# ramkp990/Truth_Recommendation_GNN

Measured on NVIDIA B200. Metric: message-passing edges/s (train step), higher is better.
Workload: dtype f32

## Files before the change

include/trg_b200.h:

```cpp
#ifndef TRG_B200_H
#define TRG_B200_H

#include <stddef.h>
#include <stdint.h>

#ifdef __cplusplus
extern "C" {
#endif

#define TRG_ABI_VERSION 4

enum { TRG_F32 = 0, TRG_BF16 = 1 };
enum {
  TRG_OK = 0,
  TRG_E_ARG = 1,
  TRG_E_WORKSPACE = 2,
  TRG_E_CUDA = 3,
  TRG_E_UNSUPPORTED = 4
};

int trg_abi_version(void);
const char* trg_last_error(void);
int64_t trg_launch_count(void);

// ... 44 lines not shown
size_t trg_edge_bce_workspace_bytes(int64_t n_users);
int trg_edge_bce_fwd(const int32_t* rowptr_u, const int32_t* col_p, const int32_t* eid,
                     const int64_t* neg_p, const void* u, const void* p,
                     int64_t n_users, int64_t n_edges, int32_t hidden, int dtype,
                     const float* wbar , float* loss_out,
                     float* c_pos, float* c_neg, void* g_u,
                     void* workspace, size_t workspace_bytes, void* stream);

int trg_edge_anchor_loss(const int32_t* rowptr, const int32_t* col, const int32_t* eid,
                         const void* anchor, const void* gathered, int64_t n_rows,
                         int64_t n_edges_scale, int32_t hidden, int dtype, int label,
                         const float* wbar, float* loss_out, float* coef_out, void* g_anchor,
                         int accumulate, int relu_gate, void* workspace, size_t workspace_bytes,
                         void* stream);

typedef struct {
  const void* a;
  const void* w;
  int32_t k;
  float alpha;
} trg_proj_term;
size_t trg_sage_proj_workspace_bytes(int32_t k_total, int32_t hidden, int dtype);
int trg_sage_proj_fwd(const trg_proj_term* terms , int32_t n_terms,
                      const float* bias ,
                      int64_t n_rows, int32_t hidden, int dtype, int relu,
                      void* out ,
                      void* workspace, size_t workspace_bytes, void* stream);

typedef struct {
  const void* w;
// ... 41 lines not shown
```

truth_recommendation_gnn_b200/_lib.py:

```python
from __future__ import annotations

import ctypes
import os

import torch

_HERE = os.path.dirname(os.path.abspath(__file__))
LIB_PATH = os.path.join(_HERE, "lib", "libtrg_b200.so")

TRG_F32, TRG_BF16 = 0, 1
ABI_VERSION = 4

_vp, _i64, _i32, _sz, _int = ctypes.c_void_p, ctypes.c_int64, ctypes.c_int32, ctypes.c_size_t, ctypes.c_int


class TrgProjTerm(ctypes.Structure):
    _fields_ = [("a", _vp), ("w", _vp), ("k", _i32), ("alpha", ctypes.c_float)]


class TrgLongRows(ctypes.Structure):
    _fields_ = [("vrowptr", _vp), ("vinfo", _vp), ("n_vrows", _i64), ("long_rows", _vp), ("long_ptr", _vp),
                ("n_long", _i64), ("partial", _vp)]


# ... 13 lines not shown
    "trg_csr_build": (_int, [_vp, _vp, _i64, _i64, _vp, _vp, _vp, _vp, _sz, _vp]),
    "trg_select_range_workspace_bytes": (_sz, [_i64]),
    "trg_select_range": (_int, [_vp, _vp, _i64, _i64, _i64, _i64, _i64, _i64, _vp, _vp, _vp, _vp, _sz, _vp]),
    "trg_sage_agg_fwd": (_int, [_vp, _vp, _vp, _i64, _i32, _int, _vp, _vp, ctypes.POINTER(TrgLongRows), _vp]),
    "trg_sage_agg_bwd": (_int, [_vp, _vp, _vp, _vp, _i64, _i32, _int, _vp, _int, _int, _vp,
                                ctypes.POINTER(TrgLongRows), _vp]),
    "trg_gather_wsum": (_int, [_vp, _vp, _vp, _vp, _vp, _vp, _i64, _i32, _int, _vp, _int, _int, _vp,
                               ctypes.POINTER(TrgLongRows), _vp]),
    "trg_rows_finish": (_int, [_vp, _int, _vp, _vp, _vp, _i64, _i32, _int, _vp, _vp]),
    "trg_peer_reduce_rows": (_int, [_vp, _i32, _i64, _int, _vp, _vp, _vp, _i64, _i32, _int, _vp, _i32, _vp]),
    "trg_edge_bce_workspace_bytes": (_sz, [_i64]),
    "trg_edge_bce_fwd": (_int, [_vp, _vp, _vp, _vp, _vp, _vp, _i64, _i64, _i32, _int, _vp, _vp,
                                _vp, _vp, _vp, _vp, _sz, _vp]),
    "trg_edge_anchor_loss": (_int, [_vp, _vp, _vp, _vp, _vp, _i64, _i64, _i32, _int, _int, _vp, _vp, _vp,
                                    _vp, _int, _int, _vp, _sz, _vp]),
    "trg_sage_proj_workspace_bytes": (_sz, [_i32, _i32, _int]),
    "trg_sage_proj_fwd": (_int, [ctypes.POINTER(TrgProjTerm), _i32, _vp, _i64, _i32, _int, _int, _vp,
                                 _vp, _sz, _vp]),
    "trg_sage_proj_bwd_input": (_int, [_vp, ctypes.POINTER(TrgProjBwdTerm), _i32, _i64, _i32, _int,
                                       _vp, _sz, _vp]),
    "trg_sage_proj_dw_workspace_bytes": (_sz, []),
    "trg_sage_proj_bwd_weight": (_int, [_vp, ctypes.POINTER(TrgProjDwTerm), _i32, _vp, _i64, _i32, _int,
                                        _vp, _sz, _vp]),
    "trg_score_topk_workspace_bytes": (_sz, [_i64, _i64, _i32, _i32]),
    "trg_score_topk": (_int, [_vp, _vp, _i64, _i64, _i32, _int, _i32, _i64, _vp, _vp, _vp, _sz, _vp]),
    "trg_score_topk_excluding": (_int, [_vp, _vp, _i64, _i64, _i32, _int, _i32, _i64, _vp, _vp, _vp, _vp, _vp,
                                        _vp, _sz, _vp]),
    "trg_topk_merge": (_int, [_vp, _vp, _i64, _i32, _i32, _i32, _vp, _vp, _vp]),
}

# ... 89 lines not shown
```

truth_recommendation_gnn_b200/csrc/csr_build.cu:

```cuda
#include <algorithm>
#include <cstdio>

#include "common.cuh"

namespace trg {
namespace {

constexpr int kThreads = 256;
constexpr int kItems = 16;
constexpr int kTile = kThreads * kItems;
constexpr int kWarps = kThreads / 32;
constexpr int kRadix = 256;

template <int NWARPS>
__device__ __forceinline__ int block_exclusive_scan(int v, int* warp_sums, int& total) {
  const int lane = threadIdx.x & 31, w = threadIdx.x >> 5;
  int inc = v;
#pragma unroll
  for (int o = 1; o < 32; o <<= 1) {
    int t = __shfl_up_sync(0xffffffffu, inc, o);
    if (lane >= o) inc += t;
  }
  if (lane == 31) warp_sums[w] = inc;
  __syncthreads();
// ... 184 lines not shown
  __shared__ int h[kRadix];
  h[threadIdx.x] = 0;
  __syncthreads();
  const int64_t base = (int64_t)blockIdx.x * kTile;
#pragma unroll
  for (int i = 0; i < kItems; ++i) {
    int64_t idx = base + (int64_t)i * kThreads + threadIdx.x;
    if (idx < n) atomicAdd(&h[(load_key<FIRST>(keys, idx) >> shift) & (kRadix - 1)], 1);
  }
  __syncthreads();
  hist[(int64_t)threadIdx.x * n_ctas + blockIdx.x] = h[threadIdx.x];
}

template <bool FIRST, bool LAST>
__global__ void __launch_bounds__(kThreads)
    radix_scatter(const void* __restrict__ keys_in, int64_t n, int shift, const int* __restrict__ gbase,
                  int n_ctas, uint2* __restrict__ pairs_out, uint32_t* __restrict__ vals_out) {
  __shared__ int wcnt[kWarps][kRadix];
  __shared__ int sbase[kRadix];
  const int lane = threadIdx.x & 31, w = threadIdx.x >> 5;
#pragma unroll
  for (int i = 0; i < kWarps; ++i) wcnt[i][threadIdx.x] = 0;
  const int64_t wbase = (int64_t)blockIdx.x * kTile + (int64_t)w * (kItems * 32);

  uint32_t key[kItems], val[kItems];
#pragma unroll
  for (int r = 0; r < kItems; ++r) {
    int64_t idx = wbase + r * 32 + lane;
    bool valid = idx < n;
    if (FIRST) {
      key[r] = valid ? load_key<true>(keys_in, idx) : 0u;
      val[r] = (uint32_t)idx;
    } else {
      const uint2 kv = valid ? ldg_pair(reinterpret_cast<const uint2*>(keys_in) + idx) : make_uint2(0u, 0u);
      key[r] = kv.x;
      val[r] = kv.y;
    }
  }
  __syncthreads();

  int rank[kItems];
#pragma unroll
  for (int r = 0; r < kItems; ++r) {
    const bool valid = wbase + r * 32 + lane < n;
    const int d = valid ? (int)((key[r] >> shift) & (kRadix - 1)) : kRadix;
    const unsigned peers = __match_any_sync(0xffffffffu, d);
    const int prev = valid ? wcnt[w][d] : 0;
// ... 31 lines not shown
                                                       const int* __restrict__ eid, int64_t n,
                                                       int* __restrict__ col) {
  int64_t i = (int64_t)blockIdx.x * blockDim.x + threadIdx.x;
  const int64_t stride = (int64_t)gridDim.x * blockDim.x;
  for (; i < n; i += stride) col[i] = (int)other[ldg_stream(eid + i)];
}

int num_passes(int64_t n_key) {
  int bits = 1;
  while (bits < 32 && ((int64_t)1 << bits) < n_key) ++bits;
  return (bits + 7) / 8;
}

struct Workspace {
  uint2* pairs[2];
  uint32_t* vals;
  int *hist, *tile_sums;
  size_t bytes;
};

Workspace carve(void* ws, int64_t e, int64_t n_key) {
  Workspace w;
  const size_t ebytes = align_up((size_t)(e > 0 ? e : 1) * 4, 256);
  const int64_t n_ctas = ceil_div<int64_t>(e > 0 ? e : 1, kTile);
  const size_t hist_bytes = align_up((size_t)kRadix * n_ctas * 4, 256);
  const int64_t scan_len = (int64_t)kRadix * n_ctas > n_key + 1 ? (int64_t)kRadix * n_ctas : n_key + 1;
  const size_t sums_bytes = align_up((size_t)ceil_div<int64_t>(scan_len, kTile) * 4 + 4, 256);
  char* p = reinterpret_cast<char*>(ws);
  w.pairs[0] = (uint2*)p; p += 2 * ebytes;
  w.pairs[1] = (uint2*)p; p += 2 * ebytes;
  w.vals = (uint32_t*)p; p += ebytes;
  w.hist = (int*)p; p += hist_bytes;
  w.tile_sums = (int*)p; p += sums_bytes;
  w.bytes = (size_t)(p - reinterpret_cast<char*>(ws));
  return w;
}

}
}

using namespace trg;

extern "C" size_t trg_csr_workspace_bytes(int64_t n_edges, int64_t n_key) {
  if (n_edges < 0 || n_key < 0) return 0;
  return carve(nullptr, n_edges, n_key).bytes;
}
// ... 20 lines not shown

  {
    int grid = (int)std::min<int64_t>(ceil_div<int64_t>(e, kThreads), (int64_t)kNumSMs * 16);
    count_keys<<<grid, kThreads, 0, st>>>((const long long*)key, e, (long long)n_key, rowptr);
    count_launch();
    TRG_LAUNCH_OK();
    int rc = exclusive_scan(rowptr, rowptr, n_key + 1, w.tile_sums, st);
    if (rc) return rc;
  }
  if (col == nullptr && eid == nullptr) return TRG_OK;

  const int passes = num_passes(n_key);
  const int n_ctas = (int)ceil_div<int64_t>(e, kTile);
  const void* kin = key;
  const uint32_t* vin = nullptr;
  for (int p = 0; p < passes; ++p) {
    const bool first = p == 0, last = p == passes - 1;
    const int shift = 8 * p;
    uint2* kout = w.pairs[p & 1];
    uint32_t* vout = eid ? (uint32_t*)eid : w.vals;
    if (first)
      radix_hist<true><<<n_ctas, kThreads, 0, st>>>(kin, e, shift, w.hist, n_ctas);
    else
      radix_hist<false><<<n_ctas, kThreads, 0, st>>>(kin, e, shift, w.hist, n_ctas);
    count_launch();
    TRG_LAUNCH_OK();
    int rc = exclusive_scan(w.hist, w.hist, (int64_t)kRadix * n_ctas, w.tile_sums, st);
    if (rc) return rc;
    if (first && last)
      radix_scatter<true, true><<<n_ctas, kThreads, 0, st>>>(kin, e, shift, w.hist, n_ctas, kout, vout);
    else if (first)
      radix_scatter<true, false><<<n_ctas, kThreads, 0, st>>>(kin, e, shift, w.hist, n_ctas, kout, vout);
    else if (last)
      radix_scatter<false, true><<<n_ctas, kThreads, 0, st>>>(kin, e, shift, w.hist, n_ctas, kout, vout);
    else
      radix_scatter<false, false><<<n_ctas, kThreads, 0, st>>>(kin, e, shift, w.hist, n_ctas, kout, vout);
    count_launch();
    TRG_LAUNCH_OK();
    kin = kout;
    vin = vout;
  }
  if (col != nullptr) {
    int grid = (int)std::min<int64_t>(ceil_div<int64_t>(e, kThreads), (int64_t)kNumSMs * 16);
    gather_col<<<grid, kThreads, 0, st>>>((const long long*)other, (const int*)vin, e, col);
    count_launch();
    TRG_LAUNCH_OK();
  }
  return TRG_OK;
}

extern "C" size_t trg_select_range_workspace_bytes(int64_t n) {
  if (n < 0) return 0;
  return align_up((size_t)(ceil_div<int64_t>(n > 0 ? n : 1, kTile) + 1) * 4, 256);
}

extern "C" int trg_select_range(const int64_t* key, const int64_t* other, int64_t n, int64_t lo, int64_t hi,
                                int64_t capacity, int64_t pad_key, int64_t pad_other, int64_t* key_out,
// ... 23 lines not shown
```

truth_recommendation_gnn_b200/csrc/edge_bce.cu:

```cuda
#include <cstdlib>

#include "common.cuh"

namespace trg {
namespace {

constexpr int kThreads = 256;

struct BceArgs {
  const int* rowptr;
  const int* col_p;
  const int* eid;
  const long long* neg_p;
  const void* u;
  const void* p;
  const float* wbar;
  float* c_pos;
  float* c_neg;
  void* g_u;
  double* partials;
  int64_t n_users;
  float inv_e;
  int row_vecs;
  int label;
// ... 186 lines not shown
#pragma unroll
              for (int i = 0; i < VPL; ++i)
                if (act[i]) {
                  float fp[kVec], fn[kVec];
                  Elem<T>::unpack(vp[q][i], fp);
                  if (TWO) Elem<T>::unpack(vn[q][i], fn);
#pragma unroll
                  for (int k = 0; k < kVec; ++k)
                    ga[i][k] = TWO ? fmaf(cpos, fp[k], fmaf(cneg, fn[k], ga[i][k])) : fmaf(cpos, fp[k], ga[i][k]);
                }
            }
          }
        }
        t += bsz;
      }
      if (want_grad && e0 + gl < e_end) {
        a.c_pos[id_cur] = my_cpos;
        if (TWO) a.c_neg[id_cur] = my_cneg;
      }
      e0 += LPR;
      cp_cur = cp_nxt; id_cur = id_nxt; cn_cur = cn_nxt;
      cp_nxt = cp_nn; id_nxt = id_nn;
    }
    while (cur < nr) flush();
  }

  double dsp = sp_sum, dsn = sn_sum;
#pragma unroll
  for (int o = 16; o > 0; o >>= 1) {
    dsp += __shfl_xor_sync(0xffffffffu, dsp, o);
    dsn += __shfl_xor_sync(0xffffffffu, dsn, o);
// ... 100 lines not shown
          cp_async16(ring_a + (uint32_t)(((slot0 + q) & (S - 1)) * 512), pb + (size_t)rid * 512 + (size_t)lane * 16);
      }
      cp_async_commit();
    };

    {
      const int id0 = load_id(e_beg), id1 = load_id(e_beg + G);
      issue(e_beg, id0, 0);
      issue(e_beg + G, id1, G);
    }
    int nid = load_id(e_beg + 2 * G);
    int slot = 0;
    for (int e_base = e_beg; e_base < e_end; e_base += G) {
      const int cnt = min(G, e_end - e_base);
      int my_id = 0;
      if (want_grad && lane < cnt) my_id = a.eid ? ldg_stream(a.eid + e_base + lane) : e_base + lane;
      cp_async_wait<1>();
      __syncwarp();
      float my_c = 0.f;
      int t = 0;
      while (t < cnt) {
        while (e_base + t >= cur_end) flush();
        const int bsz = min(cnt - t, cur_end - (e_base + t));
        uint4 vp[G];
        float v[G];
#pragma unroll
        for (int q = 0; q < G; ++q) {
          float dp = 0.f;
          if (q < bsz) {
            vp[q] = lds128_bce(ring_a + (uint32_t)(((slot + t + q) & (S - 1)) * 512));
            float fp[kVec];
// ... 30 lines not shown
          const float coef = (is_neg ? 1.f : -wbar) * sigmoid(z) * a.inv_e;
#pragma unroll
          for (int q = 0; q < G; ++q) {
            const float cq = __shfl_sync(full, coef, q * kLanesPerVal);
            if (q < bsz) {
              if (lane == t + q) my_c = cq;
              float fp[kVec];
              Elem<T>::unpack(vp[q], fp);
#pragma unroll
              for (int k = 0; k < kVec; ++k) ga[k] = fmaf(cq, fp[k], ga[k]);
            }
          }
        }
        t += bsz;
      }
      if (want_grad && lane < cnt) a.c_pos[my_id] = my_c;
      __syncwarp();
      const int nid_next = load_id(e_base + 3 * G);
      issue(e_base + 2 * G, nid, slot);
      nid = nid_next;
      slot = (slot + G) & (S - 1);
    }
    while (cur < nr) flush();
    cp_async_wait<0>();
  }

  double dsum = s_sum;
#pragma unroll
  for (int o = 16; o > 0; o >>= 1) dsum += __shfl_xor_sync(0xffffffffu, dsum, o);
  if (lane == 0) red[0][warp] = dsum;
  __syncthreads();
  if (threadIdx.x == 0) {
    double s0 = 0;
#pragma unroll
    for (int w = 0; w < kThreads / 32; ++w) s0 += red[0][w];
    const bool neg = a.label == 0;
    a.partials[2 * (size_t)blockIdx.x] = neg ? 0.0 : s0;
    a.partials[2 * (size_t)blockIdx.x + 1] = neg ? s0 : 0.0;
  }
}

__global__ void __launch_bounds__(1024) edge_bce_finish(const double* __restrict__ partials,
                                                        int64_t n_parts, const float* wbar,
                                                        double n_edges, float* loss_out) {
  __shared__ double red[2][32];
  double s0 = 0, s1 = 0;
  for (int64_t i = threadIdx.x; i < n_parts; i += 1024) {
    s0 += partials[2 * i];
    s1 += partials[2 * i + 1];
  }
#pragma unroll
  for (int o = 16; o > 0; o >>= 1) {
    s0 += __shfl_xor_sync(0xffffffffu, s0, o);
    s1 += __shfl_xor_sync(0xffffffffu, s1, o);
// ... 90 lines not shown
  edge_bce_finish<<<1, 1024, 0, st>>>(a.partials, n_blocks, wbar, (double)n_edges, loss_out);
  count_launch();
  TRG_LAUNCH_OK();
  return TRG_OK;
}

extern "C" int trg_edge_anchor_loss(const int32_t* rowptr, const int32_t* col, const int32_t* eid,
                                    const void* anchor, const void* gathered, int64_t n_rows,
                                    int64_t n_edges_scale, int32_t hidden, int dtype, int label,
                                    const float* wbar, float* loss_out, float* coef_out, void* g_anchor,
                                    int accumulate, int relu_gate, void* workspace, size_t workspace_bytes,
                                    void* stream) {
  cudaStream_t st = reinterpret_cast<cudaStream_t>(stream);
  TRG_CHECK_ARG(n_rows >= 0 && n_edges_scale >= 0, "trg_edge_anchor_loss: negative size");
  TRG_CHECK_ARG(loss_out && wbar, "trg_edge_anchor_loss: NULL loss_out/wbar");
  TRG_CHECK_ARG((coef_out == nullptr) == (g_anchor == nullptr),
                "trg_edge_anchor_loss: coef_out and g_anchor must be both NULL or both non-NULL");
  TRG_CHECK_ARG(n_rows == 0 || (rowptr && anchor), "trg_edge_anchor_loss: NULL rowptr / anchor table");
  TRG_CHECK_ARG(((uintptr_t)anchor | (uintptr_t)gathered | (uintptr_t)g_anchor) % 16 == 0,
                "trg_edge_anchor_loss: tables must be 16-byte aligned");
  TRG_CHECK_ARG(dtype == TRG_F32 || dtype == TRG_BF16, "trg_edge_anchor_loss: unknown dtype %d", dtype);
  const int es = dtype == TRG_BF16 ? 2 : 4;
  TRG_CHECK_ARG(hidden > 0 && (hidden * es) % 16 == 0,
                "trg_edge_anchor_loss: row width %d x %d bytes is not a multiple of 16 bytes", hidden, es);
  if (workspace == nullptr || workspace_bytes < trg_edge_bce_workspace_bytes(n_rows)) {
    set_error("trg_edge_anchor_loss: workspace %zu < required %zu", workspace_bytes,
              trg_edge_bce_workspace_bytes(n_rows));
    return TRG_E_WORKSPACE;
  }
  BceArgs a{};
  a.rowptr = rowptr; a.col_p = col; a.eid = eid; a.neg_p = nullptr;
  a.u = anchor; a.p = gathered; a.wbar = wbar; a.c_pos = coef_out; a.c_neg = nullptr; a.g_u = g_anchor;
// ... 17 lines not shown
    }
    count_launch();
    TRG_LAUNCH_OK();
  } else if (n_rows > 0) {
    int rc = dtype == TRG_F32 ? launch_bce<float, false>(a, &n_blocks, st, false)
                              : launch_bce<__nv_bfloat16, false>(a, &n_blocks, st, false);
    if (rc) return rc;
    count_launch();
    TRG_LAUNCH_OK();
  }
  edge_bce_finish<<<1, 1024, 0, st>>>(a.partials, n_blocks, wbar, (double)n_edges_scale, loss_out);
  count_launch();
  TRG_LAUNCH_OK();
  return TRG_OK;
}
```

truth_recommendation_gnn_b200/functional.py:

```python
from __future__ import annotations

import ctypes

import torch

from . import _lib
from .graph import CSR, RelationGraph, build_csr


def _long_rows_arg(csr: CSR, feat: int, dev, elem_size: int = 4):
    lr = csr.long_rows() if feat * elem_size >= 80 else None
    if lr is None:
        return None, None
    partial = torch.empty(lr.n_slots, feat, dtype=torch.float32, device=dev)
    s = _lib.TrgLongRows(_lib.ptr(lr.vrowptr), _lib.ptr(lr.vinfo), int(lr.vinfo.numel()), _lib.ptr(lr.long_rows),
                         _lib.ptr(lr.long_ptr), int(lr.long_rows.numel()), _lib.ptr(partial))
    return ctypes.byref(s), (s, partial)


def _check_rows(x: torch.Tensor, what: str):
    es = x.element_size()
    if x.dim() != 2 or (x.size(1) * es) % 16 != 0:
        raise _lib.TrgError(f"{what}: rows must be a multiple of 16 bytes (got shape {tuple(x.shape)}, "
                            f"{x.dtype}); pad the feature width (the reference pads to 64, inference.py:401-404)")
# ... 219 lines not shown
    ws = torch.empty(ws_bytes, dtype=torch.uint8, device=dev)
    e = ls.n_edges
    e_scale = int(getattr(ls, "n_edges_scale", e))
    rb = user_emb.size(1) * user_emb.element_size()
    nbytes = e * (2 * rb + 16 + (8 if want_grad else 0)) + ls.num_users * (rb * (2 if want_grad else 1) + 4)
    _lib.call("trg_edge_bce_fwd", nbytes, lib.trg_edge_bce_fwd,
              _lib.ptr(ls.by_user.rowptr), _lib.ptr(ls.by_user.col) if e else None,
              _lib.ptr(ls.by_user.eid) if e else None, _lib.ptr(neg_p) if e else None,
              _lib.ptr(user_emb), _lib.ptr(post_emb), ls.num_users, e_scale, user_emb.size(1),
              _lib.dtype_code(user_emb.dtype), _lib.ptr(ls.wbar), _lib.ptr(loss), _lib.ptr(c_pos),
              _lib.ptr(c_neg), _lib.ptr(g_u), _lib.ptr(ws), ws_bytes, _lib.stream())
    return loss, c_pos, c_neg, g_u


def edge_anchor_loss(csr: CSR, anchor, gathered, n_edges_scale, label, wbar, want_grad, g_anchor=None,
                     relu_gate=False, coef_in_csr_order=False):
    lib = _lib.load()
    anchor, gathered = anchor.contiguous(), gathered.contiguous()
    _check_rows(anchor, "edge_anchor_loss")
    dev = anchor.device
    loss = torch.empty(1, dtype=torch.float32, device=dev)
    coef = None
    accumulate = g_anchor is not None
    if want_grad:
        coef = torch.empty(csr.n_edges, dtype=torch.float32, device=dev)
        if g_anchor is None:
            g_anchor = torch.empty_like(anchor)
    else:
        g_anchor = None
    ws_bytes = int(lib.trg_edge_bce_workspace_bytes(csr.n_rows))
    ws = torch.empty(ws_bytes, dtype=torch.uint8, device=dev)
    e = csr.n_edges
    rb = anchor.size(1) * anchor.element_size()
    nbytes = e * (rb + 12) + csr.n_rows * (rb * (2 if want_grad else 1) + 4)
    _lib.call("trg_edge_anchor_loss", nbytes, lib.trg_edge_anchor_loss,
              _lib.ptr(csr.rowptr), _lib.ptr(csr.col) if e else None,
              _lib.ptr(csr.eid) if (e and not coef_in_csr_order) else None,
              _lib.ptr(anchor), _lib.ptr(gathered), csr.n_rows, int(n_edges_scale), anchor.size(1),
              _lib.dtype_code(anchor.dtype), 1 if label else 0, _lib.ptr(wbar), _lib.ptr(loss), _lib.ptr(coef),
              _lib.ptr(g_anchor), 1 if (accumulate and want_grad) else 0,
              1 if (relu_gate and want_grad) else 0, _lib.ptr(ws), ws_bytes, _lib.stream())
    return loss, coef, g_anchor


class LinkBCEFn(torch.autograd.Function):

    @staticmethod
    def forward(ctx, user_emb, post_emb, neg_p, ls: LinkStructure):
        want = user_emb.requires_grad or post_emb.requires_grad
        if neg_p.dtype != torch.int64 or neg_p.numel() != ls.n_edges:
            raise _lib.TrgError("neg_p must be int64 with one entry per positive edge (train_gnn.py:272)")
        if getattr(ls, "eid_long", None) is None:
            ls.eid_long = ls.by_user.eid.long()
        e_scale = int(getattr(ls, "n_edges_scale", ls.n_edges))
        bu = ls.by_user
        ctx.neg_by_post = None
        if want and ls.n_edges:
# ... 205 lines not shown
```

truth_recommendation_gnn_b200/fused_step.py:

```python
from __future__ import annotations

import torch

from . import _lib
from .functional import (edge_anchor_loss, gather_wsum, link_structure, sage_agg_bwd, sage_agg_fwd,
                         sage_proj_bwd_input, sage_proj_bwd_weight, sage_proj_fwd)
from .graph import CSR, build_csr, relation_graph
from .nn import REL_DIRECT, REL_ENGAGE, REL_SOCIAL, StackedWeightedRGCN, WeightedRGCN


def _layers(model):
    if type(model) is StackedWeightedRGCN:
        return list(model.layers)
    if type(model) is WeightedRGCN:
        return [model]
    return None


def eligible(model, x_dict) -> bool:
    layers = _layers(model)
    if layers is None or not torch.is_grad_enabled():
        return False
    xu, xp = x_dict["user"], x_dict["post"]
    if not (xu.is_cuda and xp.is_cuda) or xu.requires_grad or xp.requires_grad or xu.dtype != xp.dtype:
# ... 46 lines not shown
        hu_n = sage_proj_fwd([(mean_d, d.lin_l.weight, wd), (mean_s, s.lin_l.weight, ws), (hu, w_root, 1.0)],
                             b_user, True)
        hp_n = sage_proj_fwd([(mean_e, p.lin_l.weight, 1.0), (hp, p.lin_r.weight, 1.0)], p.lin_l.bias, True)
        saved.append((hu, hp, mean_d, mean_s, mean_e, w_root))
        hu, hp = hu_n, hp_n

    ls = link_structure(train_edge_index, interaction_type_tensor, num_users, n_p)
    if neg_ready is not None:
        torch.cuda.current_stream().wait_event(neg_ready)
    if neg_p.dtype != torch.int64 or neg_p.numel() != ls.n_edges:
        raise _lib.TrgError("neg_p must be int64 with one entry per positive edge (train_gnn.py:272)")
    if getattr(ls, "eid_long", None) is None:
        ls.eid_long = ls.by_user.eid.long()
    bu = ls.by_user
    col_neg64 = neg_p.index_select(0, ls.eid_long)
    neg_by_post = build_csr(ls.user_of_u, col_neg64, n_p, n_u, validate=False, per_step=True)
    neg_by_user = CSR(bu.rowptr, col_neg64.int(), bu.eid, bu.n_rows, bu.n_cols)
    l_pos, c_pos, dz_u = edge_anchor_loss(bu, hu, hp, ls.n_edges, 1, ls.wbar, True, None, coef_in_csr_order=True)
    l_neg, c_neg, dz_u = edge_anchor_loss(neg_by_user, hu, hp, ls.n_edges, 0, ls.wbar, True, dz_u,
                                          relu_gate=True, coef_in_csr_order=True)
    dz_p = gather_wsum(ls.by_post_u, c_pos, hu)
    gather_wsum(neg_by_post, c_neg, hu, out=dz_p, accumulate=True, relu_of=hp)
    del col_neg64
    loss = (l_pos + l_neg).reshape(())
    del neg_by_user, neg_by_post, c_pos, c_neg, hu, hp

    for li in range(len(layers) - 1, -1, -1):
        layer = layers[li]
        d, s, p = layer.msg_direct, layer.msg_social, layer.post_update
        wd, ws = float(layer.w_direct), float(layer.w_social)
        hu_in, hp_in, mean_d, mean_s, mean_e, w_root = saved.pop()
        (dw_d, dw_s, dw_root), db_u = sage_proj_bwd_weight(dz_u, [(mean_d, wd), (mean_s, ws), (hu_in, 1.0)], True)
        (dw_p, dw_pr), db_p = sage_proj_bwd_weight(dz_p, [(mean_e, 1.0), (hp_in, 1.0)], True)
        del mean_d, mean_s, mean_e
        _accum(d.lin_l.weight, dw_d)
        _accum(s.lin_l.weight, dw_s)
        _accum(d.lin_r.weight, wd * dw_root)
        _accum(s.lin_r.weight, ws * dw_root)
# ... 17 lines not shown
```

truth_recommendation_gnn_b200/graph.py:

```python
from __future__ import annotations

from collections import OrderedDict
from dataclasses import dataclass

import torch

from . import _lib


LONG_ROW_THRESHOLD = 1024


@dataclass
class LongRows:
    vrowptr: torch.Tensor
    vinfo: torch.Tensor
    long_rows: torch.Tensor
    long_ptr: torch.Tensor
    n_slots: int


@dataclass
class CSR:
    rowptr: torch.Tensor
    col: torch.Tensor
    eid: torch.Tensor
    n_rows: int
    n_cols: int
    _long: object = None

    @property
    def n_edges(self) -> int:
        return int(self.col.numel())

    def long_rows(self, threshold: int = None):
        if self._long is None:
            self._long = _split_long_rows(self, LONG_ROW_THRESHOLD if threshold is None else threshold) or False
        return self._long or None


def _split_long_rows(csr: "CSR", t: int):
# ... 10 lines not shown
    vstart = torch.cumsum(counts, 0) - counts
    k = torch.arange(n_vrows, device=rp.device) - vstart[orig]
    vrowptr = torch.empty(n_vrows + 1, dtype=torch.int32, device=rp.device)
    vrowptr[:-1] = (rp[:-1][orig] + k * t).int()
    vrowptr[-1] = csr.n_edges
    part = is_long[orig]
    slot = torch.cumsum(part.long(), 0) - 1
    vinfo = torch.where(part, -(slot + 1), orig).int()
    long_ids = is_long.nonzero().flatten()
    lp = torch.zeros(long_ids.numel() + 1, dtype=torch.long, device=rp.device)
    lp[1:] = torch.cumsum(counts[long_ids], 0)
    return LongRows(vrowptr, vinfo, long_ids.int(), lp.int(), int(lp[-1]))


def build_csr(other: torch.Tensor, key: torch.Tensor, n_key: int, n_other: int,
              validate: bool = True, per_step: bool = False) -> CSR:
    lib = _lib.load()
    if key.dtype != torch.int64 or other.dtype != torch.int64:
        raise TypeError("edge_index must be int64 (torch.long), as in the reference")
    key = key.contiguous()
    other = other.contiguous()
    e = int(key.numel())
    dev = key.device
    if validate and e > 0:
        lo_k, hi_k = int(key.min()), int(key.max())
        lo_o, hi_o = int(other.min()), int(other.max())
        if lo_k < 0 or hi_k >= n_key or lo_o < 0 or hi_o >= n_other:
            raise IndexError(f"edge_index out of range: key in [{lo_k},{hi_k}] vs {n_key}, "
                             f"other in [{lo_o},{hi_o}] vs {n_other}")
    rowptr = torch.empty(n_key + 1, dtype=torch.int32, device=dev)
    col = torch.empty(e, dtype=torch.int32, device=dev)
    eid = torch.empty(e, dtype=torch.int32, device=dev)
    ws_bytes = int(lib.trg_csr_workspace_bytes(e, n_key))
    ws = torch.empty(ws_bytes, dtype=torch.uint8, device=dev)
    _lib.call("trg_csr_build", e * 80 + 8 * (n_key + 1), lib.trg_csr_build,
              _lib.ptr(other) if e else None, _lib.ptr(key) if e else None, e, n_key, _lib.ptr(rowptr),
              _lib.ptr(col) if e else None, _lib.ptr(eid) if e else None, _lib.ptr(ws), ws_bytes,
              _lib.stream())
    return CSR(rowptr, col, eid, n_key, n_other, False if per_step else None)


class RelationGraph:

    def __init__(self, edge_index: torch.Tensor, n_src: int, n_dst: int):
        if edge_index.dim() != 2 or edge_index.size(0) != 2:
            raise ValueError("edge_index must have shape [2, E]")
        self.edge_index = edge_index
        self.n_src, self.n_dst = int(n_src), int(n_dst)
        self._fwd = None
        self._bwd = None
        self.inv_deg = None

# ... 55 lines not shown
```

Before: 2.956 billion.

## Fuse post-side link BCE gradient into one pass recomputing scores

Adds a link_post_grad kernel that walks each post's positive and negative user edges, recomputes the dot-product scores, and accumulates the weighted user rows with the ReLU gate applied in a single pass. This replaces two gather_wsum calls and removes the need to write and read per-edge coefficient arrays. The per-step negative CSR build now carries the column as the radix payload and skips the eid output and the gather_col pass. The cost is recomputing scores on the post side and a path that only applies to 512-byte rows.

Measured after the change: 3.023 billion (median of 6 runs). 1.02x the previous value.

```diff
diff --git a/include/trg_b200.h b/include/trg_b200.h
--- a/include/trg_b200.h
+++ b/include/trg_b200.h
@@ -82,6 +82,12 @@
                          int accumulate, int relu_gate, void* workspace, size_t workspace_bytes,
                          void* stream);
 
+int trg_link_post_grad(const int32_t* pos_rowptr, const int32_t* pos_col, const int32_t* neg_rowptr,
+                       const int32_t* neg_col, const void* hp, const void* hu, int64_t n_posts,
+                       int64_t n_edges_scale, int32_t hidden, int dtype, const float* wbar ,
+                       void* dz_p ,
+                       const trg_long_rows* long_rows , void* stream);
+
 typedef struct {
   const void* a;
   const void* w;
diff --git a/truth_recommendation_gnn_b200/_lib.py b/truth_recommendation_gnn_b200/_lib.py
--- a/truth_recommendation_gnn_b200/_lib.py
+++ b/truth_recommendation_gnn_b200/_lib.py
@@ -51,6 +51,8 @@
                                 _vp, _vp, _vp, _vp, _sz, _vp]),
     "trg_edge_anchor_loss": (_int, [_vp, _vp, _vp, _vp, _vp, _i64, _i64, _i32, _int, _int, _vp, _vp, _vp,
                                     _vp, _int, _int, _vp, _sz, _vp]),
+    "trg_link_post_grad": (_int, [_vp, _vp, _vp, _vp, _vp, _vp, _i64, _i64, _i32, _int, _vp, _vp,
+                                  ctypes.POINTER(TrgLongRows), _vp]),
     "trg_sage_proj_workspace_bytes": (_sz, [_i32, _i32, _int]),
     "trg_sage_proj_fwd": (_int, [ctypes.POINTER(TrgProjTerm), _i32, _vp, _i64, _i32, _int, _int, _vp,
                                  _vp, _sz, _vp]),
diff --git a/truth_recommendation_gnn_b200/csrc/csr_build.cu b/truth_recommendation_gnn_b200/csrc/csr_build.cu
--- a/truth_recommendation_gnn_b200/csrc/csr_build.cu
+++ b/truth_recommendation_gnn_b200/csrc/csr_build.cu
@@ -222,8 +222,9 @@
 
 template <bool FIRST, bool LAST>
 __global__ void __launch_bounds__(kThreads)
-    radix_scatter(const void* __restrict__ keys_in, int64_t n, int shift, const int* __restrict__ gbase,
-                  int n_ctas, uint2* __restrict__ pairs_out, uint32_t* __restrict__ vals_out) {
+    radix_scatter(const void* __restrict__ keys_in, const long long* __restrict__ payload, int64_t n, int shift,
+                  const int* __restrict__ gbase, int n_ctas, uint2* __restrict__ pairs_out,
+                  uint32_t* __restrict__ vals_out) {
   __shared__ int wcnt[kWarps][kRadix];
   __shared__ int sbase[kRadix];
   const int lane = threadIdx.x & 31, w = threadIdx.x >> 5;
@@ -238,7 +239,7 @@
     bool valid = idx < n;
     if (FIRST) {
       key[r] = valid ? load_key<true>(keys_in, idx) : 0u;
-      val[r] = (uint32_t)idx;
+      val[r] = payload ? (valid ? (uint32_t)ldg_stream(payload + idx) : 0u) : (uint32_t)idx;
     } else {
       const uint2 kv = valid ? ldg_pair(reinterpret_cast<const uint2*>(keys_in) + idx) : make_uint2(0u, 0u);
       key[r] = kv.x;
@@ -300,7 +301,6 @@
 
 struct Workspace {
   uint2* pairs[2];
-  uint32_t* vals;
   int *hist, *tile_sums;
   size_t bytes;
 };
@@ -315,7 +315,6 @@
   char* p = reinterpret_cast<char*>(ws);
   w.pairs[0] = (uint2*)p; p += 2 * ebytes;
   w.pairs[1] = (uint2*)p; p += 2 * ebytes;
-  w.vals = (uint32_t*)p; p += ebytes;
   w.hist = (int*)p; p += hist_bytes;
   w.tile_sums = (int*)p; p += sums_bytes;
   w.bytes = (size_t)(p - reinterpret_cast<char*>(ws));
@@ -366,11 +365,12 @@
   const int n_ctas = (int)ceil_div<int64_t>(e, kTile);
   const void* kin = key;
   const uint32_t* vin = nullptr;
+  const long long* payload = eid ? nullptr : (const long long*)other;
   for (int p = 0; p < passes; ++p) {
     const bool first = p == 0, last = p == passes - 1;
     const int shift = 8 * p;
     uint2* kout = w.pairs[p & 1];
-    uint32_t* vout = eid ? (uint32_t*)eid : w.vals;
+    uint32_t* vout = eid ? (uint32_t*)eid : (uint32_t*)col;
     if (first)
       radix_hist<true><<<n_ctas, kThreads, 0, st>>>(kin, e, shift, w.hist, n_ctas);
     else
@@ -380,19 +380,19 @@
     int rc = exclusive_scan(w.hist, w.hist, (int64_t)kRadix * n_ctas, w.tile_sums, st);
     if (rc) return rc;
     if (first && last)
-      radix_scatter<true, true><<<n_ctas, kThreads, 0, st>>>(kin, e, shift, w.hist, n_ctas, kout, vout);
+      radix_scatter<true, true><<<n_ctas, kThreads, 0, st>>>(kin, payload, e, shift, w.hist, n_ctas, kout, vout);
     else if (first)
-      radix_scatter<true, false><<<n_ctas, kThreads, 0, st>>>(kin, e, shift, w.hist, n_ctas, kout, vout);
+      radix_scatter<true, false><<<n_ctas, kThreads, 0, st>>>(kin, payload, e, shift, w.hist, n_ctas, kout, vout);
     else if (last)
-      radix_scatter<false, true><<<n_ctas, kThreads, 0, st>>>(kin, e, shift, w.hist, n_ctas, kout, vout);
+      radix_scatter<false, true><<<n_ctas, kThreads, 0, st>>>(kin, payload, e, shift, w.hist, n_ctas, kout, vout);
     else
-      radix_scatter<false, false><<<n_ctas, kThreads, 0, st>>>(kin, e, shift, w.hist, n_ctas, kout, vout);
+      radix_scatter<false, false><<<n_ctas, kThreads, 0, st>>>(kin, payload, e, shift, w.hist, n_ctas, kout, vout);
     count_launch();
     TRG_LAUNCH_OK();
     kin = kout;
     vin = vout;
   }
-  if (col != nullptr) {
+  if (col != nullptr && eid != nullptr) {
     int grid = (int)std::min<int64_t>(ceil_div<int64_t>(e, kThreads), (int64_t)kNumSMs * 16);
     gather_col<<<grid, kThreads, 0, st>>>((const long long*)other, (const int*)vin, e, col);
     count_launch();
diff --git a/truth_recommendation_gnn_b200/csrc/edge_bce.cu b/truth_recommendation_gnn_b200/csrc/edge_bce.cu
--- a/truth_recommendation_gnn_b200/csrc/edge_bce.cu
+++ b/truth_recommendation_gnn_b200/csrc/edge_bce.cu
@@ -224,7 +224,7 @@
         }
         t += bsz;
       }
-      if (want_grad && e0 + gl < e_end) {
+      if (a.c_pos && e0 + gl < e_end) {
         a.c_pos[id_cur] = my_cpos;
         if (TWO) a.c_neg[id_cur] = my_cneg;
       }
@@ -355,7 +355,7 @@
     for (int e_base = e_beg; e_base < e_end; e_base += G) {
       const int cnt = min(G, e_end - e_base);
       int my_id = 0;
-      if (want_grad && lane < cnt) my_id = a.eid ? ldg_stream(a.eid + e_base + lane) : e_base + lane;
+      if (a.c_pos && lane < cnt) my_id = a.eid ? ldg_stream(a.eid + e_base + lane) : e_base + lane;
       cp_async_wait<1>();
       __syncwarp();
       float my_c = 0.f;
@@ -416,7 +416,7 @@
         }
         t += bsz;
       }
-      if (want_grad && lane < cnt) a.c_pos[my_id] = my_c;
+      if (a.c_pos && lane < cnt) a.c_pos[my_id] = my_c;
       __syncwarp();
       const int nid_next = load_id(e_base + 3 * G);
       issue(e_base + 2 * G, nid, slot);
@@ -440,6 +440,311 @@
     a.partials[2 * (size_t)blockIdx.x] = neg ? 0.0 : s0;
     a.partials[2 * (size_t)blockIdx.x + 1] = neg ? s0 : 0.0;
   }
+}
+
+struct PostGradArgs {
+  const int* pos_rowptr;
+  const int* vinfo;
+  const int* pos_col;
+  const int* neg_rowptr;
+  const int* neg_col;
+  const void* hp;
+  const void* hu;
+  const float* wbar;
+  void* dz_p;
+  float* partial;
+  const int* long_rows;
+  const int* long_ptr;
+  int n_long;
+  int64_t n_vrows;
+  float inv_e;
+};
+
+template <typename T>
+constexpr int kPgG = sizeof(T) == 4 ? 4 : 2;
+constexpr int kPgSlots = 12;
+constexpr int kPgR = 4;
+constexpr int kPgBytes = (kThreads / 32) * (kPgSlots + 1) * 512;
+
+template <typename T, int G>
+__device__ __forceinline__ float batch_scores(const uint4* vr, int bsz, const float* af) {
+  constexpr int kVec = Elem<T>::kVec;
+  const int lane = threadIdx.x & 31;
+  float v[G];
+#pragma unroll
+  for (int q = 0; q < G; ++q) {
+    float dp = 0.f;
+    if (q < bsz) {
+      float f[kVec];
+      Elem<T>::unpack(vr[q], f);
+#pragma unroll
+      for (int k = 0; k < kVec; ++k) dp = fmaf(f[k], af[k], dp);
+    }
+    v[q] = dp;
+  }
+  int nv = G;
+#pragma unroll
+  for (int o = 16; o > 0; o >>= 1) {
+    if (nv > 1) {
+      nv >>= 1;
+#pragma unroll
+      for (int i = 0; i < G / 2; ++i) {
+        if (i < nv) {
+          const bool hi = (lane & o) != 0;
+          const float send = hi ? v[i] : v[i + nv];
+          const float keep = hi ? v[i + nv] : v[i];
+          v[i] = keep + __shfl_xor_sync(0xffffffffu, send, o);
+        }
+      }
+    } else {
+      v[0] += __shfl_xor_sync(0xffffffffu, v[0], o);
+    }
+  }
+  return v[0];
+}
+
+__device__ __forceinline__ float link_coef(float s, bool neg, float wbar, float inv_e) {
+  const float z = neg ? s : -s;
+  return (neg ? 1.f : -wbar) * sigmoid(z) * inv_e;
+}
+
+template <typename T>
+__device__ __forceinline__ void post_grad_store(char* dst, const float* an, const float* pr, const float* af) {
+  constexpr int kVec = Elem<T>::kVec;
+  float o[kVec];
+#pragma unroll
+  for (int k = 0; k < kVec; ++k) {
+    o[k] = an[k] + pr[k];
+    o[k] = af[k] > 0.f ? o[k] : 0.f;
+  }
+  stg_stream(dst, Elem<T>::pack(o));
+}
+
+template <typename T, bool VIRT>
+__global__ void __launch_bounds__(kThreads, 4) link_post_grad(const PostGradArgs a) {
+  constexpr int kVec = Elem<T>::kVec;
+  constexpr int R = kPgR, G = kPgG<T>, S = kPgSlots, NG = S / G;
+  constexpr int kLanesPerVal = 32 / G;
+  constexpr unsigned full = 0xffffffffu;
+  extern __shared__ __align__(16) unsigned char ring_raw[];
+  const int lane = threadIdx.x & 31, warp = threadIdx.x >> 5;
+  const int64_t r0 = ((int64_t)blockIdx.x * (kThreads / 32) + warp) * R;
+  if (r0 >= a.n_vrows) return;
+  const uint32_t smem0 = static_cast<uint32_t>(__cvta_generic_to_shared(ring_raw));
+  const uint32_t ring_a = smem0 + (uint32_t)(warp * S * 512 + lane * 16);
+  const uint32_t pos_a = smem0 + (uint32_t)(((kThreads / 32) * S + warp) * 512 + lane * 16);
+  const int nr = (int)((a.n_vrows - r0) < (int64_t)R ? (a.n_vrows - r0) : (int64_t)R);
+  const char* hpb = reinterpret_cast<const char*>(a.hp);
+  const char* hub = reinterpret_cast<const char*>(a.hu);
+  const float wbar = __ldg(a.wbar);
+
+  int pb = 0, np = 0, nb = 0, nn = 0, info = 0, arow = 0;
+  if (lane < nr) {
+    pb = ldg_stream(a.pos_rowptr + r0 + lane);
+    np = ldg_stream(a.pos_rowptr + r0 + lane + 1) - pb;
+    info = VIRT ? ldg_stream(a.vinfo + r0 + lane) : (int)(r0 + lane);
+    if (info >= 0) {
+      nb = ldg_stream(a.neg_rowptr + info);
+      nn = ldg_stream(a.neg_rowptr + info + 1) - nb;
+      arow = info;
+    } else {
+      const int slot = -(info + 1);
+      int lo = 0, hi = a.n_long - 1;
+      while (lo < hi) {
+        const int mid = (lo + hi + 1) >> 1;
+        if (__ldg(a.long_ptr + mid) <= slot) lo = mid; else hi = mid - 1;
+      }
+      arow = __ldg(a.long_rows + lo);
+    }
+  }
+  int inc = np + nn;
+#pragma unroll
+  for (int o = 1; o < R; o <<= 1) {
+    const int t = __shfl_up_sync(full, inc, o);
+    if (lane >= o) inc += t;
+  }
+  const int e_end = __shfl_sync(full, inc, nr - 1);
+  const int cs = lane < nr ? inc - (np + nn) : e_end;
+
+  auto row_lane = [&](int m, int v) { return __shfl_sync(full, v, m); };
+  auto load_id = [&](int ebase) -> int {
+    const int e = ebase + lane;
+    int r = 0;
+#pragma unroll
+    for (int m = 1; m < R; ++m)
+      if (e >= row_lane(m, cs)) r = m;
+    const int off = e - row_lane(r, cs);
+    const int npr = row_lane(r, np), pbr = row_lane(r, pb), nbr = row_lane(r, nb);
+    if (lane >= G || e >= e_end) return 0;
+    return off < npr ? ldg_stream(a.pos_col + pbr + off) : ldg_stream(a.neg_col + nbr + (off - npr));
+  };
+  auto issue = [&](int ebase, int ids, int slot0) {
+#pragma unroll
+    for (int q = 0; q < G; ++q) {
+      const int rid = __shfl_sync(full, ids, q);
+      if (ebase + q < e_end)
+        cp_async16(ring_a + (uint32_t)((slot0 + q) * 512), hub + (size_t)rid * 512 + (size_t)lane * 16);
+    }
+    cp_async_commit();
+  };
+
+  float af[kVec], acc[kVec];
+#pragma unroll
+  for (int k = 0; k < kVec; ++k) acc[k] = 0.f;
+  Elem<T>::unpack(ldg_row(hpb + (size_t)row_lane(0, arow) * 512 + (size_t)lane * 16), af);
+  uint4 a_nxt = make_uint4(0, 0, 0, 0);
+  {
+    const int ar1 = row_lane(1, arow);
+    if (nr > 1) a_nxt = ldg_row(hpb + (size_t)ar1 * 512 + (size_t)lane * 16);
+  }
+  int cur = 0;
+  int cur_end = row_lane(1, cs);
+  int pos_end = row_lane(0, np);
+  bool in_neg = false;
+
+  auto flush = [&]() {
+    const int inf = row_lane(cur, info);
+    if (VIRT && inf < 0) {
+      float* pbp = a.partial + (size_t)(-(inf + 1)) * (32 * kVec) + (size_t)lane * kVec;
+#pragma unroll
+      for (int k = 0; k < kVec; ++k) pbp[k] = acc[k];
+    } else {
+      float pr[kVec], an[kVec];
+      if (in_neg) {
+        Elem<T>::unpack(lds128_bce(pos_a), pr);
+#pragma unroll
+        for (int k = 0; k < kVec; ++k) an[k] = acc[k];
+      } else {
+        Elem<T>::unpack(Elem<T>::pack(acc), pr);
+#pragma unroll
+        for (int k = 0; k < kVec; ++k) an[k] = 0.f;
+      }
+      post_grad_store<T>(reinterpret_cast<char*>(a.dz_p) + (size_t)inf * 512 + (size_t)lane * 16, an, pr, af);
+    }
+#pragma unroll
+    for (int k = 0; k < kVec; ++k) acc[k] = 0.f;
+    in_neg = false;
+    ++cur;
+    pos_end = cur_end + row_lane(cur, np);
+    cur_end = row_lane(cur + 1, cs);
+    Elem<T>::unpack(a_nxt, af);
+    const int arn = row_lane(cur + 1, arow);
+    if (cur + 1 < nr) a_nxt = ldg_row(hpb + (size_t)arn * 512 + (size_t)lane * 16);
+  };
+
+#pragma unroll
+  for (int g = 0; g < NG; ++g) issue(g * G, load_id(g * G), g * G);
+  int nid = load_id(NG * G);
+  int slot = 0;
+  for (int e_base = 0; e_base < e_end; e_base += G) {
+    const int cnt = min(G, e_end - e_base);
+    cp_async_wait<NG - 1>();
+    __syncwarp();
+    int t = 0;
+    while (t < cnt) {
+      const int e = e_base + t;
+      while (e >= cur_end) flush();
+      if (!in_neg && e >= pos_end) {
+        const uint4 pk = Elem<T>::pack(acc);
+        asm volatile("st.shared.v4.u32 [%0], {%1,%2,%3,%4};" ::"r"(pos_a), "r"(pk.x), "r"(pk.y), "r"(pk.z),
+                     "r"(pk.w) : "memory");
+#pragma unroll
+        for (int k = 0; k < kVec; ++k) acc[k] = 0.f;
+        in_neg = true;
+      }
+      const int bsz = min(cnt - t, (in_neg ? cur_end : pos_end) - e);
+      uint4 vr[G];
+#pragma unroll
+      for (int q = 0; q < G; ++q)
+        if (q < bsz) vr[q] = lds128_bce(ring_a + (uint32_t)((slot + t + q) * 512));
+      const float s = batch_scores<T, G>(vr, bsz, af);
+      const float coef = link_coef(s, in_neg, wbar, a.inv_e);
+#pragma unroll
+      for (int q = 0; q < G; ++q) {
+        const float cq = __shfl_sync(full, coef, q * kLanesPerVal);
+        if (q < bsz) {
+          float f[kVec];
+          Elem<T>::unpack(vr[q], f);
+#pragma unroll
+          for (int k = 0; k < kVec; ++k) acc[k] = fmaf(cq, f[k], acc[k]);
+        }
+      }
+      t += bsz;
+    }
+    __syncwarp();
+    const int nid_next = load_id(e_base + (NG + 1) * G);
+    issue(e_base + NG * G, nid, slot);
+    nid = nid_next;
+    slot = slot + G == S ? 0 : slot + G;
+  }
+  while (cur < nr) flush();
+  cp_async_wait<0>();
+}
+
+template <typename T>
+__global__ void __launch_bounds__(32) link_post_combine(const PostGradArgs a) {
+  constexpr int kVec = Elem<T>::kVec;
+  constexpr int G = kPgG<T>, kLanesPerVal = 32 / G;
+  const int lane = threadIdx.x;
+  const int row = a.long_rows[blockIdx.x];
+  const int s0 = a.long_ptr[blockIdx.x], s1 = a.long_ptr[blockIdx.x + 1];
+  const float wbar = __ldg(a.wbar);
+  float af[kVec], ap[kVec], an[kVec];
+  Elem<T>::unpack(ldg_row(reinterpret_cast<const char*>(a.hp) + (size_t)row * 512 + (size_t)lane * 16), af);
+#pragma unroll
+  for (int k = 0; k < kVec; ++k) {
+    float s = 0.f;
+    for (int sl = s0; sl < s1; ++sl) s += a.partial[(size_t)sl * (32 * kVec) + (size_t)lane * kVec + k];
+    ap[k] = s;
+    an[k] = 0.f;
+  }
+  const int nb = a.neg_rowptr[row], ne = a.neg_rowptr[row + 1];
+  const char* hub = reinterpret_cast<const char*>(a.hu);
+  for (int e = nb; e < ne; e += G) {
+    const int bsz = min(G, ne - e);
+    const int my = lane < bsz ? ldg_stream(a.neg_col + e + lane) : 0;
+    uint4 vr[G];
+#pragma unroll
+    for (int q = 0; q < G; ++q) {
+      const int u = __shfl_sync(0xffffffffu, my, q);
+      if (q < bsz) vr[q] = ldg_row(hub + (size_t)u * 512 + (size_t)lane * 16);
+    }
+    const float coef = link_coef(batch_scores<T, G>(vr, bsz, af), true, wbar, a.inv_e);
+#pragma unroll
+    for (int q = 0; q < G; ++q) {
+      const float cq = __shfl_sync(0xffffffffu, coef, q * kLanesPerVal);
+      if (q < bsz) {
+        float f[kVec];
+        Elem<T>::unpack(vr[q], f);
+#pragma unroll
+        for (int k = 0; k < kVec; ++k) an[k] = fmaf(cq, f[k], an[k]);
+      }
+    }
+  }
+  float pr[kVec];
+  Elem<T>::unpack(Elem<T>::pack(ap), pr);
+  post_grad_store<T>(reinterpret_cast<char*>(a.dz_p) + (size_t)row * 512 + (size_t)lane * 16, an, pr, af);
+}
+
+template <typename T>
+int launch_post_grad(const PostGradArgs& a, cudaStream_t st) {
+  static SmemAttrState attr_plain, attr_virt;
+  const int64_t grid = ceil_div<int64_t>(a.n_vrows, (int64_t)(kThreads / 32) * kPgR);
+  if (a.vinfo) {
+    TRG_CUDA(ensure_dyn_smem(link_post_grad<T, true>, kPgBytes, attr_virt));
+    link_post_grad<T, true><<<(unsigned)grid, kThreads, kPgBytes, st>>>(a);
+  } else {
+    TRG_CUDA(ensure_dyn_smem(link_post_grad<T, false>, kPgBytes, attr_plain));
+    link_post_grad<T, false><<<(unsigned)grid, kThreads, kPgBytes, st>>>(a);
+  }
+  count_launch();
+  TRG_LAUNCH_OK();
+  if (a.vinfo && a.n_long > 0) {
+    link_post_combine<T><<<(unsigned)a.n_long, 32, 0, st>>>(a);
+    count_launch();
+    TRG_LAUNCH_OK();
+  }
+  return TRG_OK;
 }
 
 __global__ void __launch_bounds__(1024) edge_bce_finish(const double* __restrict__ partials,
@@ -560,8 +865,7 @@
   cudaStream_t st = reinterpret_cast<cudaStream_t>(stream);
   TRG_CHECK_ARG(n_rows >= 0 && n_edges_scale >= 0, "trg_edge_anchor_loss: negative size");
   TRG_CHECK_ARG(loss_out && wbar, "trg_edge_anchor_loss: NULL loss_out/wbar");
-  TRG_CHECK_ARG((coef_out == nullptr) == (g_anchor == nullptr),
-                "trg_edge_anchor_loss: coef_out and g_anchor must be both NULL or both non-NULL");
+  TRG_CHECK_ARG(coef_out == nullptr || g_anchor != nullptr, "trg_edge_anchor_loss: coef_out needs g_anchor");
   TRG_CHECK_ARG(n_rows == 0 || (rowptr && anchor), "trg_edge_anchor_loss: NULL rowptr / anchor table");
   TRG_CHECK_ARG(((uintptr_t)anchor | (uintptr_t)gathered | (uintptr_t)g_anchor) % 16 == 0,
                 "trg_edge_anchor_loss: tables must be 16-byte aligned");
@@ -609,3 +913,32 @@
   TRG_LAUNCH_OK();
   return TRG_OK;
 }
+
+extern "C" int trg_link_post_grad(const int32_t* pos_rowptr, const int32_t* pos_col, const int32_t* neg_rowptr,
+                                  const int32_t* neg_col, const void* hp, const void* hu, int64_t n_posts,
+                                  int64_t n_edges_scale, int32_t hidden, int dtype, const float* wbar, void* dz_p,
+                                  const trg_long_rows* lr, void* stream) {
+  TRG_CHECK_ARG(n_posts >= 0 && n_edges_scale >= 0, "trg_link_post_grad: negative size");
+  if (n_posts == 0) return TRG_OK;
+  TRG_CHECK_ARG(pos_rowptr && neg_rowptr && hp && hu && wbar && dz_p, "trg_link_post_grad: NULL argument");
+  TRG_CHECK_ARG(((uintptr_t)hp | (uintptr_t)hu | (uintptr_t)dz_p) % 16 == 0,
+                "trg_link_post_grad: tables must be 16-byte aligned");
+  TRG_CHECK_ARG(dtype == TRG_F32 || dtype == TRG_BF16, "trg_link_post_grad: unknown dtype %d", dtype);
+  const int es = dtype == TRG_BF16 ? 2 : 4;
+  if (hidden * es != 512) {
+    set_error("trg_link_post_grad: rows must be 512 bytes (fp32 H=128, bf16 H=256), got %d x %d", hidden, es);
+    return TRG_E_UNSUPPORTED;
+  }
+  PostGradArgs a{};
+  a.pos_rowptr = pos_rowptr; a.pos_col = pos_col; a.neg_rowptr = neg_rowptr; a.neg_col = neg_col;
+  a.hp = hp; a.hu = hu; a.wbar = wbar; a.dz_p = dz_p; a.n_vrows = n_posts;
+  a.inv_e = n_edges_scale > 0 ? (float)(1.0 / (double)n_edges_scale) : 0.f;
+  if (lr && lr->n_long > 0) {
+    TRG_CHECK_ARG(lr->vrowptr && lr->vinfo && lr->long_rows && lr->long_ptr && lr->partial,
+                  "trg_link_post_grad: incomplete trg_long_rows");
+    a.pos_rowptr = lr->vrowptr; a.vinfo = lr->vinfo; a.n_vrows = lr->n_vrows;
+    a.partial = lr->partial; a.long_rows = lr->long_rows; a.long_ptr = lr->long_ptr; a.n_long = (int)lr->n_long;
+  }
+  cudaStream_t st = reinterpret_cast<cudaStream_t>(stream);
+  return dtype == TRG_F32 ? launch_post_grad<float>(a, st) : launch_post_grad<__nv_bfloat16>(a, st);
+}
diff --git a/truth_recommendation_gnn_b200/functional.py b/truth_recommendation_gnn_b200/functional.py
--- a/truth_recommendation_gnn_b200/functional.py
+++ b/truth_recommendation_gnn_b200/functional.py
@@ -257,7 +257,7 @@
 
 
 def edge_anchor_loss(csr: CSR, anchor, gathered, n_edges_scale, label, wbar, want_grad, g_anchor=None,
-                     relu_gate=False, coef_in_csr_order=False):
+                     relu_gate=False, coef_in_csr_order=False, want_coef=True):
     lib = _lib.load()
     anchor, gathered = anchor.contiguous(), gathered.contiguous()
     _check_rows(anchor, "edge_anchor_loss")
@@ -266,7 +266,8 @@
     coef = None
     accumulate = g_anchor is not None
     if want_grad:
-        coef = torch.empty(csr.n_edges, dtype=torch.float32, device=dev)
+        if want_coef:
+            coef = torch.empty(csr.n_edges, dtype=torch.float32, device=dev)
         if g_anchor is None:
             g_anchor = torch.empty_like(anchor)
     else:
@@ -275,15 +276,36 @@
     ws = torch.empty(ws_bytes, dtype=torch.uint8, device=dev)
     e = csr.n_edges
     rb = anchor.size(1) * anchor.element_size()
-    nbytes = e * (rb + 12) + csr.n_rows * (rb * (2 if want_grad else 1) + 4)
+    nbytes = e * (rb + 4 + (8 if coef is not None else 0)) + csr.n_rows * (rb * (2 if want_grad else 1) + 4)
     _lib.call("trg_edge_anchor_loss", nbytes, lib.trg_edge_anchor_loss,
               _lib.ptr(csr.rowptr), _lib.ptr(csr.col) if e else None,
-              _lib.ptr(csr.eid) if (e and not coef_in_csr_order) else None,
+              _lib.ptr(csr.eid) if (e and coef is not None and not coef_in_csr_order) else None,
               _lib.ptr(anchor), _lib.ptr(gathered), csr.n_rows, int(n_edges_scale), anchor.size(1),
               _lib.dtype_code(anchor.dtype), 1 if label else 0, _lib.ptr(wbar), _lib.ptr(loss), _lib.ptr(coef),
               _lib.ptr(g_anchor), 1 if (accumulate and want_grad) else 0,
               1 if (relu_gate and want_grad) else 0, _lib.ptr(ws), ws_bytes, _lib.stream())
     return loss, coef, g_anchor
+
+
+def link_post_grad(by_post: CSR, neg_by_post: CSR, hp, hu, n_edges_scale, wbar):
+    lib = _lib.load()
+    hp, hu = hp.contiguous(), hu.contiguous()
+    if hp.dtype != hu.dtype or hp.size(1) != hu.size(1) or hp.size(1) * hp.element_size() != 512:
+        raise _lib.TrgError("link_post_grad: hp and hu must share dtype and have 512-byte rows")
+    if neg_by_post.n_rows != by_post.n_rows or by_post.n_rows != hp.size(0):
+        raise _lib.TrgError("link_post_grad: both structures must have one row per post")
+    dz_p = torch.empty_like(hp)
+    if by_post.n_rows:
+        rb = 512
+        e = by_post.n_edges + neg_by_post.n_edges
+        nbytes = e * (rb + 4) + by_post.n_rows * (2 * rb + 8)
+        lr, keep = _long_rows_arg(by_post, hp.size(1), hp.device, hp.element_size())
+        _lib.call("trg_link_post_grad", nbytes, lib.trg_link_post_grad,
+                  _lib.ptr(by_post.rowptr), _lib.ptr(by_post.col) if by_post.n_edges else None,
+                  _lib.ptr(neg_by_post.rowptr), _lib.ptr(neg_by_post.col) if neg_by_post.n_edges else None,
+                  _lib.ptr(hp), _lib.ptr(hu), by_post.n_rows, int(n_edges_scale), hp.size(1),
+                  _lib.dtype_code(hp.dtype), _lib.ptr(wbar), _lib.ptr(dz_p), lr, _lib.stream())
+    return dz_p
 
 
 class LinkBCEFn(torch.autograd.Function):
diff --git a/truth_recommendation_gnn_b200/fused_step.py b/truth_recommendation_gnn_b200/fused_step.py
--- a/truth_recommendation_gnn_b200/fused_step.py
+++ b/truth_recommendation_gnn_b200/fused_step.py
@@ -3,8 +3,8 @@
 import torch
 
 from . import _lib
-from .functional import (edge_anchor_loss, gather_wsum, link_structure, sage_agg_bwd, sage_agg_fwd,
-                         sage_proj_bwd_input, sage_proj_bwd_weight, sage_proj_fwd)
+from .functional import (edge_anchor_loss, gather_wsum, link_post_grad, link_structure, sage_agg_bwd,
+                         sage_agg_fwd, sage_proj_bwd_input, sage_proj_bwd_weight, sage_proj_fwd)
 from .graph import CSR, build_csr, relation_graph
 from .nn import REL_DIRECT, REL_ENGAGE, REL_SOCIAL, StackedWeightedRGCN, WeightedRGCN
 
@@ -84,14 +84,20 @@
         ls.eid_long = ls.by_user.eid.long()
     bu = ls.by_user
     col_neg64 = neg_p.index_select(0, ls.eid_long)
-    neg_by_post = build_csr(ls.user_of_u, col_neg64, n_p, n_u, validate=False, per_step=True)
+    one_pass = hu.size(1) * hu.element_size() == 512
+    neg_by_post = build_csr(ls.user_of_u, col_neg64, n_p, n_u, validate=False, per_step=True,
+                            want_eid=not one_pass)
     neg_by_user = CSR(bu.rowptr, col_neg64.int(), bu.eid, bu.n_rows, bu.n_cols)
-    l_pos, c_pos, dz_u = edge_anchor_loss(bu, hu, hp, ls.n_edges, 1, ls.wbar, True, None, coef_in_csr_order=True)
+    del col_neg64
+    l_pos, c_pos, dz_u = edge_anchor_loss(bu, hu, hp, ls.n_edges, 1, ls.wbar, True, None, coef_in_csr_order=True,
+                                          want_coef=not one_pass)
     l_neg, c_neg, dz_u = edge_anchor_loss(neg_by_user, hu, hp, ls.n_edges, 0, ls.wbar, True, dz_u,
-                                          relu_gate=True, coef_in_csr_order=True)
-    dz_p = gather_wsum(ls.by_post_u, c_pos, hu)
-    gather_wsum(neg_by_post, c_neg, hu, out=dz_p, accumulate=True, relu_of=hp)
-    del col_neg64
+                                          relu_gate=True, coef_in_csr_order=True, want_coef=not one_pass)
+    if one_pass:
+        dz_p = link_post_grad(ls.by_post, neg_by_post, hp, hu, ls.n_edges, ls.wbar)
+    else:
+        dz_p = gather_wsum(ls.by_post_u, c_pos, hu)
+        gather_wsum(neg_by_post, c_neg, hu, out=dz_p, accumulate=True, relu_of=hp)
     loss = (l_pos + l_neg).reshape(())
     del neg_by_user, neg_by_post, c_pos, c_neg, hu, hp
 
diff --git a/truth_recommendation_gnn_b200/graph.py b/truth_recommendation_gnn_b200/graph.py
--- a/truth_recommendation_gnn_b200/graph.py
+++ b/truth_recommendation_gnn_b200/graph.py
@@ -24,7 +24,7 @@
 class CSR:
     rowptr: torch.Tensor
     col: torch.Tensor
-    eid: torch.Tensor
+    eid: object
     n_rows: int
     n_cols: int
     _long: object = None
@@ -65,7 +65,7 @@
 
 
 def build_csr(other: torch.Tensor, key: torch.Tensor, n_key: int, n_other: int,
-              validate: bool = True, per_step: bool = False) -> CSR:
+              validate: bool = True, per_step: bool = False, want_eid: bool = True) -> CSR:
     lib = _lib.load()
     if key.dtype != torch.int64 or other.dtype != torch.int64:
         raise TypeError("edge_index must be int64 (torch.long), as in the reference")
@@ -81,12 +81,12 @@
                              f"other in [{lo_o},{hi_o}] vs {n_other}")
     rowptr = torch.empty(n_key + 1, dtype=torch.int32, device=dev)
     col = torch.empty(e, dtype=torch.int32, device=dev)
-    eid = torch.empty(e, dtype=torch.int32, device=dev)
+    eid = torch.empty(e, dtype=torch.int32, device=dev) if want_eid else None
     ws_bytes = int(lib.trg_csr_workspace_bytes(e, n_key))
     ws = torch.empty(ws_bytes, dtype=torch.uint8, device=dev)
     _lib.call("trg_csr_build", e * 80 + 8 * (n_key + 1), lib.trg_csr_build,
               _lib.ptr(other) if e else None, _lib.ptr(key) if e else None, e, n_key, _lib.ptr(rowptr),
-              _lib.ptr(col) if e else None, _lib.ptr(eid) if e else None, _lib.ptr(ws), ws_bytes,
+              _lib.ptr(col) if e else None, _lib.ptr(eid) if (e and want_eid) else None, _lib.ptr(ws), ws_bytes,
               _lib.stream())
     return CSR(rowptr, col, eid, n_key, n_other, False if per_step else None)
 
```
